# NVIDIA/DALI

Measured on NVIDIA B200. Metric: images/sec decode+resize+CMN (batch 256, 1080p JPEG), higher is better.
Workload: dtype u8

## Files before the change

dali_b200/csrc/common.cuh:

```cuda
#ifndef DALI_B200_CSRC_COMMON_CUH_
#define DALI_B200_CSRC_COMMON_CUH_

#include <cuda_runtime.h>
#include <cuda_fp16.h>
#include <stdint.h>
#include <atomic>
#include <cstdio>
#include <cstdarg>
#include <string>
#include <vector>
#include "../../include/dali_b200.h"

namespace dalib200 {

void SetLastError(const char *fmt, ...);
extern std::atomic<uint64_t> g_launch_count;
inline void CountLaunch(int n = 1) { g_launch_count.fetch_add(n, std::memory_order_relaxed); }

#define DB_CHECK_ARG(cond, ...)                                   \
  do { if (!(cond)) { ::dalib200::SetLastError(__VA_ARGS__); return DALIB200_ERROR_INVALID_ARGUMENT; } } while (0)

#define DB_CUDA(call)                                                                           \
  do { cudaError_t e__ = (call); if (e__ != cudaSuccess) {                                      \
    ::dalib200::SetLastError("CUDA error %s at %s:%d (%s)", cudaGetErrorName(e__), __FILE__, __LINE__, \
// ... 61 lines not shown

__device__ __forceinline__ float u8_to_float(uint32_t b) { return __uint_as_float(0x4B000000u | b) - 8388608.0f; }

template <typename T> struct OutConv;
template <> struct OutConv<float> {
  __device__ __forceinline__ static float cvt(float v) { return v; }
};
template <> struct OutConv<uint16_t> {
  __device__ __forceinline__ static uint16_t cvt(float v) { return float2half_ties_away(v); }
};

__device__ __forceinline__ float mul_rn(float a, float b) { return __fmul_rn(a, b); }
__device__ __forceinline__ float add_rn(float a, float b) { return __fadd_rn(a, b); }
__device__ __forceinline__ float sub_rn(float a, float b) { return __fsub_rn(a, b); }

__device__ __forceinline__ uint32_t ld_nc_u32(const uint32_t *p) {
  uint32_t v;
  asm volatile("ld.global.nc.u32 %0, [%1];" : "=r"(v) : "l"(p));
  return v;
}

__device__ __forceinline__ uint32_t smem_u32(const void *p) { return (uint32_t)__cvta_generic_to_shared(p); }
__device__ __forceinline__ uint32_t lds_u32(uint32_t a) { uint32_t v; asm volatile("ld.shared.u32 %0, [%1];" : "=r"(v) : "r"(a)); return v; }
__device__ __forceinline__ uint32_t lds_u16(uint32_t a) { unsigned short v; asm volatile("ld.shared.u16 %0, [%1];" : "=h"(v) : "r"(a)); return v; }
__device__ __forceinline__ uint32_t lds_u8(uint32_t a) { uint32_t v; asm volatile("ld.shared.u8 %0, [%1];" : "=r"(v) : "r"(a)); return v; }
__device__ __forceinline__ void sts_u32(uint32_t a, uint32_t v) { asm volatile("st.shared.u32 [%0], %1;" :: "r"(a), "r"(v) : "memory"); }
__device__ __forceinline__ void sts_u16(uint32_t a, uint32_t v) { asm volatile("st.shared.u16 [%0], %1;" :: "r"(a), "h"((unsigned short)v) : "memory"); }

__device__ __forceinline__ void mbar_init(uint64_t *bar, uint32_t count) {
  asm volatile("mbarrier.init.shared::cta.b64 [%0], %1;" :: "r"(smem_u32(bar)), "r"(count) : "memory");
}
__device__ __forceinline__ void mbar_expect_tx(uint64_t *bar, uint32_t bytes) {
  asm volatile("mbarrier.arrive.expect_tx.shared::cta.b64 _, [%0], %1;" :: "r"(smem_u32(bar)), "r"(bytes) : "memory");
}
__device__ __forceinline__ void mbar_arrive(uint64_t *bar) {
  asm volatile("mbarrier.arrive.shared::cta.b64 _, [%0];" :: "r"(smem_u32(bar)) : "memory");
}
__device__ __forceinline__ void mbar_wait(uint64_t *bar, uint32_t parity) {
  asm volatile("{\n\t.reg .pred p;\n\tWAIT_%=:\n\tmbarrier.try_wait.parity.shared::cta.b64 p, [%0], %1;\n\t@p bra DONE_%=;\n\tbra WAIT_%=;\n\tDONE_%=:\n\t}"
               :: "r"(smem_u32(bar)), "r"(parity) : "memory");
}
__device__ __forceinline__ void mbar_wait_backoff(uint64_t *bar, uint32_t parity) {
  uint32_t done = 0;
  for (;;) {
    asm volatile("{\n\t.reg .pred p;\n\tmbarrier.try_wait.parity.shared::cta.b64 p, [%1], %2;\n\tselp.u32 %0, 1, 0, p;\n\t}"
                 : "=r"(done) : "r"(smem_u32(bar)), "r"(parity) : "memory");
    if (done) break;
// ... 35 lines not shown
```

dali_b200/csrc/jpeg.cu:

```cuda
#include "common.cuh"
#include <algorithm>
#include <cstring>
#include <map>
#include <thread>

namespace dalib200 {

constexpr int kDcLutBits = 9, kAcLutBits = 11;
constexpr int kDcLutSize = 1 << kDcLutBits, kAcLutSize = 1 << kAcLutBits;
constexpr int kLutWords = 2 * kDcLutSize + 2 * kAcLutSize;
constexpr int kSyncThreads = 256;
constexpr int kChunkBytes = 4096;
constexpr int kMaxBlocksPerMcu = 10;
constexpr int kMaxLog2Sub = 10;

constexpr int kLongLut = 512;
struct HuffSlow {
  int32_t maxcode[18];
  int32_t valoff[18];
  uint8_t vals[256];
  int32_t long_base, long_n;
  uint16_t long_lut[kLongLut];
};

struct TableSet {
  uint32_t lut[kLutWords];
  uint16_t lut16[kLutWords];
  HuffSlow slow[4];
};
__host__ __device__ inline int LutOffset(int t) { return t < 2 ? t * kDcLutSize : 2 * kDcLutSize + (t - 2) * kAcLutSize; }

struct QuantSet { uint16_t q[4][64]; };

struct JpegImage {
  uint8_t *out;
  int32_t width, height, ncomp;
  int32_t hs[3], vs[3], hmax, vmax;
  int32_t mcux, mcuy, bpm;
  int32_t blk_comp[kMaxBlocksPerMcu];
  int32_t blk_dc[kMaxBlocksPerMcu], blk_ac[kMaxBlocksPerMcu];
  int32_t blk_x[kMaxBlocksPerMcu], blk_y[kMaxBlocksPerMcu];
  int32_t tq[3];
  int32_t restart_interval;
  int32_t table_set, quant_set;
  int32_t unit_begin, unit_end;
  int32_t subseq_begin;
  int32_t nsub;
  int32_t block_begin;
  int32_t wblock_begin;
// ... 182 lines not shown
    uint32_t *cw32 = reinterpret_cast<uint32_t *>(clean) + (out_base >> 2);
    for (uint32_t wd = threadIdx.x; wd < nwords; wd += blockDim.x) {
      const uint32_t v = obuf[wd];
      const bool full = (wd > 0 || head == 0) && (wd + 1 < nwords || tailb == 0);
      if (full) {
        cw32[wd] = __byte_perm(v, 0u, 0x0123);
      } else {
        const uint32_t lo = wd == 0 ? head : 0u, hi = (wd + 1 == nwords && tailb) ? tailb : 4u;
        for (uint32_t b = lo; b < hi; b++) reinterpret_cast<uint8_t *>(cw32 + wd)[3u - b] = (uint8_t)(v >> (8 * b));
      }
    }
    if (c0 + kChunkBytes >= u.raw_len) {
      const uint32_t e0 = out_base + total, e1 = u.clean_off + ((u.raw_len + 32u + 15u) & ~15u);
      for (uint32_t q = e0 + threadIdx.x; q < e1; q += blockDim.x) clean[(q & ~3u) | (3u - (q & 3u))] = 0;
    }
    __syncthreads();
  }
}

struct SmemSrc {
  uint32_t base; int lsw;
  __device__ __forceinline__ uint32_t load(uint32_t g) const { return lds_u32(base + ((g ^ ((g >> lsw) & 31u)) << 2)); }
};
struct SmemLut { uint32_t base; __device__ __forceinline__ uint32_t load(uint32_t i) const { return lds_u32(base + (i << 2)); } };
struct GlobalLut { const uint32_t *p; __device__ __forceinline__ uint32_t load(uint32_t i) const { return __ldg(p + i); } };
template <int STRIDE> struct SmemTbl { uint32_t base; __device__ __forceinline__ uint32_t load(int c) const { return lds_u32(base + (uint32_t)c * (STRIDE * 4u)); } };
struct GlobalSrc {
  const uint32_t *w;
  __device__ __forceinline__ uint32_t load(uint32_t g) const { return __ldg(w + g); }
};

template <class Src>
struct BitWindow {
  uint32_t hi, lo, g;
  int avail;
  __device__ __forceinline__ void init(const Src &s, uint32_t word, uint32_t sh) {
    const uint32_t w0 = s.load(word), w1 = s.load(word + 1);
    hi = __funnelshift_l(w1, w0, sh);
    lo = w1 << sh;
    avail = 64 - (int)sh;
    g = word + 2;
  }
  __device__ __forceinline__ void consume(const Src &s, uint32_t e) {
    hi = __funnelshift_l(lo, hi, e);
    lo = __funnelshift_l(0u, lo, e);
    avail -= (int)(e & 31u);
    const uint32_t w = s.load(g);
    const bool need = avail < 32;
    const uint32_t a = (uint32_t)avail & 31u;
    hi |= (need ? w : 0u) >> a;
    lo = need ? (w << ((32u - a) & 31u)) : lo;
    avail += need ? 32 : 0;
    g += need ? 1u : 0u;
  }
};

constexpr uint64_t kStateMask = (1ull << 42) - 1;
constexpr uint32_t kMaxChainLen = 4095;
__device__ __forceinline__ uint64_t pack_state(uint32_t p, int c, int z, uint32_t cnt = 0, uint32_t t = 0) {
  return (uint64_t)p | ((uint64_t)(uint32_t)c << 32) | ((uint64_t)(uint32_t)z << 36) | ((uint64_t)min(cnt, 1023u) << 42) | ((uint64_t)t << 52);
}
__device__ __forceinline__ uint32_t state_count(uint64_t s) { return (uint32_t)(s >> 42) & 1023u; }

__device__ __forceinline__ uint32_t make_entry(uint32_t len, uint32_t sym, bool is_dc) {
  const uint32_t s = sym & 15u, r = sym >> 4;
  const uint32_t adv = is_dc ? 1u : (s == 0 ? (r == 15u ? 16u : 64u) : r + 1u);
  return (len + s) | (s << 8) | (len << 12) | (adv << 20);
}

__device__ __forceinline__ uint32_t make_entry16(uint32_t len, uint32_t sym, bool is_dc) {
  const uint32_t s = sym & 15u, r = sym >> 4;
  const uint32_t adv = is_dc ? 1u : (s == 0 ? (r == 15u ? 16u : 64u) : r + 1u);
  return (len + s) | (s << 5) | (adv << 9);
}

__device__ __noinline__ uint32_t slow_lookup(const HuffSlow *__restrict__ slow, uint32_t toff, uint32_t hi, bool is_dc) {
  const int tbl = toff < 2u * kDcLutSize ? (int)(toff / kDcLutSize) : 2 + (int)((toff - 2u * kDcLutSize) / kAcLutSize);
  const HuffSlow *sl = slow + tbl;
  const int32_t code16 = (int32_t)(hi >> 16);
  if (sl->long_n > 0) {
    const int idx = min(max(code16 - sl->long_base, 0), sl->long_n - 1);
    const uint32_t e = sl->long_lut[idx];
    return e ? e : 16u;
  }
  uint32_t len = (is_dc ? kDcLutBits : kAcLutBits) + 1;
  while (len <= 16 && code16 >= sl->maxcode[len]) len++;
  uint32_t sym = 0;
  if (len > 16) len = 16;
  else sym = sl->vals[(sl->valoff[len] + (code16 >> (16 - len))) & 0xFF];
  return len | (sym << 8);
}
__device__ __forceinline__ uint32_t slow_symbol(const HuffSlow *__restrict__ slow, uint32_t toff, uint32_t hi, bool is_dc) {
  const uint32_t ls = slow_lookup(slow, toff, hi, is_dc);
  return make_entry(ls & 0xFFu, ls >> 8, is_dc);
}
__device__ __forceinline__ uint32_t slow_symbol16(const HuffSlow *__restrict__ slow, uint32_t toff, uint32_t hi, bool is_dc) {
  const uint32_t ls = slow_lookup(slow, toff, hi, is_dc);
  return make_entry16(ls & 0xFFu, ls >> 8, is_dc);
}

template <class Src, class Lut, class Tbl>
__device__ __forceinline__ void decode_span(const Src &src, BitWindow<Src> &win, const Lut &lut, const HuffSlow *__restrict__ slow,
                                            const Tbl &tbl, int bpm, uint32_t &pos, uint32_t end, int &c, int &z, uint32_t &nb) {
  uint32_t tb12 = tbl.load(c);
  while (pos < end) {
    const uint32_t e_ac = lut.load((tb12 >> 16) + (win.hi >> (32 - kAcLutBits)));
    const bool is_dc = z == 0;
    uint32_t e = e_ac;
    if (is_dc) e = lut.load((tb12 & 0xFFFFu) + (win.hi >> (32 - kDcLutBits)));
    if (__builtin_expect(e == 0, 0)) e = slow_symbol(slow, is_dc ? (tb12 & 0xFFFFu) : (tb12 >> 16), win.hi, is_dc);
    const uint32_t tb = e & 31u, adv = e >> 20;
    win.consume(src, e);
    pos += tb;
    z += (int)adv;
    const bool endb = z >= 64;
    const int c1 = c + 1 == bpm ? 0 : c + 1;
    nb += endb ? 1u : 0u;
    c = endb ? c1 : c;
    z = endb ? 0 : z;
    if (endb) tb12 = tbl.load(c);
  }
}

__device__ __forceinline__ int find_unit_by_subseq(const JpegUnit *u, int ub, int ue, int j) {
  int lo = ub, hi = ue - 1;
  while (lo < hi) {
    int mid = (lo + hi + 1) >> 1;
    if (u[mid].first_subseq <= j) lo = mid; else hi = mid - 1;
  }
  return lo;
}

struct HuffCtx {
  const JpegImage *images; int nimages;
  const int32_t *block_image;
  const int32_t *wblock_image;
  const JpegUnit *units;
  const uint32_t *unit_clean_len;
  const TableSet *tables;
  const uint8_t *clean;
  uint64_t *s_state;
  uint32_t *s_n;
  int16_t *coef;
  int16_t *dc;
  int log2_sub;
  int32_t *status;
  uint32_t *unit_nblk;
  uint4 *chains[3];
  uint32_t *chain_count;
};

__device__ __forceinline__ uint32_t tbl_word(const JpegImage &im, int b) {
  return (uint32_t)LutOffset(im.blk_dc[b]) | ((uint32_t)LutOffset(im.blk_ac[b]) << 16);
}

struct SyncSmem {
  uint32_t *lut, *sw, *cnt, *tbl, *col_end, *blkbuf;
  uint64_t *exitst;
  const uint8_t **colptr;
  uint8_t *zig, *col_cont;
  HuffSlow *slow;
};
constexpr int kMaxLookAheadCols = 8;
__host__ __device__ inline int look_ahead_cols(int log2_sub) { return 256 >> (log2_sub - 3); }
__host__ __device__ inline size_t sync_sw_words(int log2_sub) { return (size_t)(kSyncThreads + look_ahead_cols(log2_sub)) << (log2_sub - 5); }
__host__ __device__ inline size_t sync_smem_bytes(int log2_sub, bool with_block_buffers) {
  return kLutWords * 4 + sync_sw_words(log2_sub) * 4 + kSyncThreads * 8  + (kSyncThreads + kMaxLookAheadCols) * 8  +
         kSyncThreads * 4 * 2  + 16 * 4  + 64  + kSyncThreads  + 4 * sizeof(HuffSlow) +
         (with_block_buffers ? (size_t)kSyncThreads * 128 : 0) ;
}
__device__ __forceinline__ SyncSmem carve_sync_smem(uint32_t *base, int log2_sub) {
  SyncSmem s;
  s.lut = base;
  s.sw = s.lut + kLutWords;
  s.exitst = reinterpret_cast<uint64_t *>(s.sw + sync_sw_words(log2_sub));
  s.colptr = reinterpret_cast<const uint8_t **>(s.exitst + kSyncThreads);
  s.cnt = reinterpret_cast<uint32_t *>(s.colptr + kSyncThreads + kMaxLookAheadCols);
  s.col_end = s.cnt + kSyncThreads;
  s.tbl = s.col_end + kSyncThreads;
  s.zig = reinterpret_cast<uint8_t *>(s.tbl + 16);
  s.col_cont = s.zig + 64;
  s.slow = reinterpret_cast<HuffSlow *>(s.col_cont + kSyncThreads);
  s.blkbuf = reinterpret_cast<uint32_t *>(s.slow + 4);
  return s;
}

struct SubGeom { bool valid; int ui; uint32_t jl, nsub_eff, clean_bits; int64_t g; };

__device__ __forceinline__ SubGeom sync_block_prologue(const HuffCtx &cx, const JpegImage &im, const SyncSmem &sm) {
  const int lsw = cx.log2_sub - 5;
  {
    const uint4 *src = reinterpret_cast<const uint4 *>(cx.tables[im.table_set].lut);
    uint4 *dst = reinterpret_cast<uint4 *>(sm.lut);
    for (int i = threadIdx.x; i < kLutWords / 4; i += blockDim.x) dst[i] = __ldg(src + i);
    if (threadIdx.x < kMaxBlocksPerMcu) sm.tbl[threadIdx.x] = tbl_word(im, threadIdx.x);
    if (threadIdx.x < 64) sm.zig[threadIdx.x] = c_zigzag[threadIdx.x];
    const uint32_t *ssrc = reinterpret_cast<const uint32_t *>(cx.tables[im.table_set].slow);
    uint32_t *sdst = reinterpret_cast<uint32_t *>(sm.slow);
    for (int i = threadIdx.x; i < (int)(4 * sizeof(HuffSlow) / 4); i += blockDim.x) sdst[i] = __ldg(ssrc + i);
  }
  SubGeom sg;
  const int j = (blockIdx.x - im.block_begin) * kSyncThreads + threadIdx.x;
  sg.valid = j < im.nsub;
  sg.ui = 0; sg.jl = 0; sg.nsub_eff = 0; sg.clean_bits = 0;
  sg.g = (int64_t)im.subseq_begin + j;
  const uint8_t *ptr = nullptr;
  if (sg.valid) {
    sg.ui = im.unit_end - im.unit_begin == 1 ? im.unit_begin : find_unit_by_subseq(cx.units, im.unit_begin, im.unit_end, j);
    const JpegUnit &u = cx.units[sg.ui];
    sg.clean_bits = cx.unit_clean_len[sg.ui] * 8u;
    sg.nsub_eff = (sg.clean_bits + (1u << cx.log2_sub) - 1) >> cx.log2_sub;
    sg.jl = (uint32_t)(j - u.first_subseq);
    sg.valid = sg.jl < sg.nsub_eff;
    if (sg.valid) ptr = cx.clean + u.clean_off + ((size_t)sg.jl << (cx.log2_sub - 3));
  }
  sm.colptr[threadIdx.x] = ptr;
  sm.col_end[threadIdx.x] = min((sg.jl + 1) << cx.log2_sub, sg.clean_bits);
// ... 49 lines not shown
      const uint32_t x = threadIdx.x + 1;
      nb = 0;
      decode_span(src, win, lut, slow, tbl, im.bpm, pos, sm.col_end[x], c, z, nb);
      const uint64_t ns = pack_state(pos, c, z);
      const bool same = sm.exitst[x] == ns;
      sm.exitst[x] = ns; sm.cnt[x] = nb;
      if (!same && sm.col_cont[x]) push_chain(cx, 0, pos, c, z, 2u, sg.g + 2, img_i);
    }
  }
  __syncthreads();
  if (sg.valid) {
    const uint32_t t = threadIdx.x > 0 && sm.col_cont[threadIdx.x - 1] ? 1u : 0u;
    cx.s_state[sg.g] = sm.exitst[threadIdx.x] | ((uint64_t)min(sm.cnt[threadIdx.x], 1023u) << 42) | ((uint64_t)t << 52);
  }
}

constexpr int kTailThreads = 256;
constexpr int kTailColWords = 36;
struct ColSrc {
  uint32_t base;
  __device__ __forceinline__ uint32_t load(uint32_t g) const { return lds_u32(base + g * (kTailThreads * 4u)); }
};

__device__ __forceinline__ void walk_chain(const HuffCtx &cx, const uint4 rec, int out_list, int max_visits, const uint32_t *s_lut,
                                           const HuffSlow *s_slow, int s_table_set, uint32_t *col, uint32_t *tblcol) {
  const int img_i = (int)rec.w;
  const JpegImage &im = cx.images[img_i];
  int64_t g = rec.z;
  const int j = (int)(g - im.subseq_begin);
  const int ui = im.unit_end - im.unit_begin == 1 ? im.unit_begin : find_unit_by_subseq(cx.units, im.unit_begin, im.unit_end, j);
  const JpegUnit &u = cx.units[ui];
  const uint32_t clean_bits = cx.unit_clean_len[ui] * 8u;
  const uint32_t nsub_eff = (clean_bits + (1u << cx.log2_sub) - 1) >> cx.log2_sub;
  uint32_t jl = (uint32_t)(j - u.first_subseq);
#pragma unroll
  for (int b = 0; b < kMaxBlocksPerMcu; b++) tblcol[b * kTailThreads] = tbl_word(im, b);
  const bool shared_tables = im.table_set == s_table_set;
  uint32_t pos = rec.x, t = rec.y >> 16;
  int c = (int)(rec.y & 0xFF), z = (int)((rec.y >> 8) & 0xFF);
  const int sub_words = 1 << (cx.log2_sub - 5);
  for (int visit = 0;;) {
    uint32_t nb = 0;
    const uint32_t end = min((jl + 1) << cx.log2_sub, clean_bits);
    if (shared_tables && sub_words + 4 <= kTailColWords) {
      const uint4 *p4 = reinterpret_cast<const uint4 *>(cx.clean + u.clean_off + ((size_t)jl << (cx.log2_sub - 3)));
      for (int q = 0; q < sub_words / 4 + 1; q++) {
        const uint4 v = __ldg(p4 + q);
        col[(4 * q + 0) * kTailThreads] = v.x; col[(4 * q + 1) * kTailThreads] = v.y;
        col[(4 * q + 2) * kTailThreads] = v.z; col[(4 * q + 3) * kTailThreads] = v.w;
      }
      const ColSrc src{smem_u32(col)};
      const uint32_t rel = pos - (jl << cx.log2_sub);
      BitWindow<ColSrc> win;
      win.init(src, rel >> 5, rel & 31u);
      decode_span(src, win, SmemLut{smem_u32(s_lut)}, s_slow, SmemTbl<kTailThreads>{smem_u32(tblcol)}, im.bpm, pos, end, c, z, nb);
    } else {
      const GlobalSrc src{reinterpret_cast<const uint32_t *>(cx.clean + u.clean_off)};
      BitWindow<GlobalSrc> win;
      win.init(src, pos >> 5, pos & 31u);
      decode_span(src, win, GlobalLut{cx.tables[im.table_set].lut}, cx.tables[im.table_set].slow, SmemTbl<kTailThreads>{smem_u32(tblcol)},
                  im.bpm, pos, end, c, z, nb);
    }
    const uint64_t ns = pack_state(pos, c, z, nb, t);
    const uint64_t old = atomicMax(reinterpret_cast<unsigned long long *>(cx.s_state + g), (unsigned long long)ns);
    if ((uint32_t)(old >> 52) >= t) break;
    if (((old ^ ns) & kStateMask) == 0) break;
    if (jl + 1 >= nsub_eff || t >= kMaxChainLen) break;
    g++; jl++; t++;
    if (++visit >= max_visits) { push_chain(cx, out_list, pos, c, z, t, g, img_i); break; }
  }
}

__global__ void __launch_bounds__(kTailThreads) huff_sync_walk_kernel(HuffCtx cx, int in_list, int out_list, int max_visits) {
  extern __shared__ __align__(16) uint32_t tsm[];
  const uint32_t n = cx.chain_count[in_list];
  if (blockIdx.x * blockDim.x >= n) return;
  uint32_t *s_lut = tsm;
  HuffSlow *s_slow = reinterpret_cast<HuffSlow *>(s_lut + kLutWords);
  uint32_t *col = reinterpret_cast<uint32_t *>(s_slow + 4) + threadIdx.x;
  uint32_t *tblcol = reinterpret_cast<uint32_t *>(s_slow + 4) + kTailColWords * kTailThreads + threadIdx.x;
  const int s_table_set = cx.images[0].table_set;
  {
    const uint4 *src = reinterpret_cast<const uint4 *>(cx.tables[s_table_set].lut);
    uint4 *dst = reinterpret_cast<uint4 *>(s_lut);
    for (int i = threadIdx.x; i < kLutWords / 4; i += blockDim.x) dst[i] = __ldg(src + i);
    const uint32_t *ssrc = reinterpret_cast<const uint32_t *>(cx.tables[s_table_set].slow);
    uint32_t *sdst = reinterpret_cast<uint32_t *>(s_slow);
    for (int i = threadIdx.x; i < (int)(4 * sizeof(HuffSlow) / 4); i += blockDim.x) sdst[i] = __ldg(ssrc + i);
  }
  __syncthreads();
  const uint32_t gtid = blockIdx.x * blockDim.x + threadIdx.x, gsize = gridDim.x * blockDim.x;
  for (uint32_t i = gtid; i < n; i += gsize) walk_chain(cx, cx.chains[in_list][i], out_list, max_visits, s_lut, s_slow, s_table_set, col, tblcol);
}

__global__ void __launch_bounds__(1024) huff_scan_kernel(HuffCtx cx) {
  __shared__ uint32_t warp_tot[32];
  __shared__ uint32_t carry;
  const JpegImage &im = cx.images[blockIdx.x];
  const uint32_t sub_bits = 1u << cx.log2_sub;
  for (int ui = im.unit_begin; ui < im.unit_end; ui++) {
    const JpegUnit &u = cx.units[ui];
    const uint32_t clean_bits = cx.unit_clean_len[ui] * 8u;
    const uint32_t nsub_eff = (clean_bits + sub_bits - 1) >> cx.log2_sub;
    const int64_t g0 = (int64_t)im.subseq_begin + u.first_subseq;
    __syncthreads();
    if (threadIdx.x == 0) carry = 0;
    __syncthreads();
    for (uint32_t base = 0; base < nsub_eff; base += blockDim.x) {
// ... 3 lines not shown
      for (int o = 1; o < 32; o <<= 1) { uint32_t x = __shfl_up_sync(0xffffffffu, incl, o); if ((threadIdx.x & 31) >= o) incl += x; }
      if ((threadIdx.x & 31) == 31) warp_tot[threadIdx.x >> 5] = incl;
      __syncthreads();
      uint32_t woff = 0, tot = 0;
      for (int w = 0; w < (int)(blockDim.x >> 5); w++) { if (w < (int)(threadIdx.x >> 5)) woff += warp_tot[w]; tot += warp_tot[w]; }
      if (i < nsub_eff) cx.s_n[g0 + i] = carry + woff + incl - v;
      __syncthreads();
      if (threadIdx.x == 0) carry += tot;
      __syncthreads();
    }
    if (threadIdx.x == 0) {
      if ((int64_t)carry * 64 < u.nslots) cx.status[blockIdx.x] = 1;
      cx.unit_nblk[ui] = (uint32_t)min((int64_t)carry, u.nslots >> 6);
    }
  }
}

constexpr int kWriteThreads = 384;
struct WriteSmem {
  uint16_t *lut; uint32_t *sw, *tbl, *blkbuf; uint8_t *zig; HuffSlow *slow; const uint8_t **colptr;
};
__host__ __device__ inline size_t write_sw_words(int log2_sub) { return (size_t)(kWriteThreads + look_ahead_cols(log2_sub)) << (log2_sub - 5); }
__host__ __device__ inline size_t write_smem_bytes(int log2_sub) {
  return kLutWords * 2 + write_sw_words(log2_sub) * 4 + 16 * 4  + 64  + (size_t)kWriteThreads * 128;
}
__device__ __forceinline__ WriteSmem carve_write_smem(uint32_t *base, int log2_sub) {
  WriteSmem s;
  s.lut = reinterpret_cast<uint16_t *>(base);
  s.sw = base + kLutWords / 2;
  s.tbl = s.sw + write_sw_words(log2_sub);
  s.zig = reinterpret_cast<uint8_t *>(s.tbl + 16);
  s.slow = nullptr;
  s.blkbuf = reinterpret_cast<uint32_t *>(s.zig + 64);
  s.colptr = reinterpret_cast<const uint8_t **>(s.blkbuf);
  return s;
}

__global__ void __launch_bounds__(kWriteThreads) huff_write_kernel(HuffCtx cx) {
  extern __shared__ __align__(16) uint32_t hsm[];
  const WriteSmem sm = carve_write_smem(hsm, cx.log2_sub);
  const JpegImage &im = cx.images[cx.wblock_image[blockIdx.x]];
  const int lsw = cx.log2_sub - 5;
  {
    const uint4 *src = reinterpret_cast<const uint4 *>(cx.tables[im.table_set].lut16);
    uint4 *dst = reinterpret_cast<uint4 *>(sm.lut);
    for (int i = threadIdx.x; i < kLutWords * 2 / 16; i += blockDim.x) dst[i] = __ldg(src + i);
    if (threadIdx.x < kMaxBlocksPerMcu) sm.tbl[threadIdx.x] = tbl_word(im, threadIdx.x);
    if (threadIdx.x < 64) sm.zig[threadIdx.x] = c_zigzag[threadIdx.x];
  }
  SubGeom sg;
  {
    const int j = (blockIdx.x - im.wblock_begin) * kWriteThreads + threadIdx.x;
    sg.valid = j < im.nsub;
    sg.ui = 0; sg.jl = 0; sg.nsub_eff = 0; sg.clean_bits = 0;
    sg.g = (int64_t)im.subseq_begin + j;
    const uint8_t *ptr = nullptr;
    if (sg.valid) {
      sg.ui = im.unit_end - im.unit_begin == 1 ? im.unit_begin : find_unit_by_subseq(cx.units, im.unit_begin, im.unit_end, j);
      const JpegUnit &u = cx.units[sg.ui];
      sg.clean_bits = cx.unit_clean_len[sg.ui] * 8u;
      sg.nsub_eff = (sg.clean_bits + (1u << cx.log2_sub) - 1) >> cx.log2_sub;
      sg.jl = (uint32_t)(j - u.first_subseq);
      sg.valid = sg.jl < sg.nsub_eff;
      if (sg.valid) ptr = cx.clean + u.clean_off + ((size_t)sg.jl << (cx.log2_sub - 3));
    }
    sm.colptr[threadIdx.x] = ptr;
    const int la_cols = look_ahead_cols(cx.log2_sub);
    if (threadIdx.x == kWriteThreads - 1)
      for (int q = 1; q <= la_cols; q++) sm.colptr[kWriteThreads - 1 + q] = ptr ? ptr + ((size_t)q << (cx.log2_sub - 3)) : nullptr;
    __syncthreads();
    const int cpc = 1 << (cx.log2_sub - 7);
    for (int ch = threadIdx.x; ch < (kWriteThreads + la_cols) * cpc; ch += blockDim.x) {
      const int col = ch / cpc, o = ch - col * cpc;
      const uint8_t *p = sm.colptr[col];
      if (p) {
        const uint4 v = __ldg(reinterpret_cast<const uint4 *>(p) + o);
        const uint32_t g = ((uint32_t)col << lsw) + 4u * o, x = (uint32_t)col & 31u;
        sm.sw[(g + 0) ^ x] = v.x; sm.sw[(g + 1) ^ x] = v.y; sm.sw[(g + 2) ^ x] = v.z; sm.sw[(g + 3) ^ x] = v.w;
      }
    }
    __syncthreads();
  }
  const HuffSlow *slow = cx.tables[im.table_set].slow;
  const SmemSrc src{smem_u32(sm.sw), lsw};
  const uint32_t lane = threadIdx.x & 31u;
  const uint32_t a_lut = smem_u32(sm.lut), a_tbl = smem_u32(sm.tbl), a_zig = smem_u32(sm.zig);
  const uint32_t a_wbuf = smem_u32(sm.blkbuf) + (threadIdx.x & ~31u) * 128u;
  const uint32_t a_mybuf = a_wbuf + lane * 128u;
#pragma unroll
  for (int j = 0; j < 32; j++) sts_u32(a_mybuf + 4u * j, 0u);
  __syncwarp();
  uint32_t pos = 0, nb = 0, end = 0, hard_end = 0, blk0 = 0, blk_limit = 0;
  int c = 0, z = 0;
  bool active = sg.valid;
  if (active) {
    const JpegUnit &u = cx.units[sg.ui];
    if (sg.jl > 0) {
      const uint64_t prev = cx.s_state[sg.g - 1];
      pos = (uint32_t)prev; c = (int)((prev >> 32) & 15u); z = (int)((prev >> 36) & 63u);
    }
    end = min((sg.jl + 1) << cx.log2_sub, sg.clean_bits);
    hard_end = sg.clean_bits;
    const uint32_t ublk = (uint32_t)(u.slot_base >> 6);
    blk0 = ublk + cx.s_n[sg.g];
    blk_limit = ublk + (uint32_t)(u.nslots >> 6);
    active = pos < end && blk0 < blk_limit;
  }
  bool own = z == 0;
  BitWindow<SmemSrc> win;
  {
    const uint32_t rel = active ? pos - (sg.jl << cx.log2_sub) : 0u;
    win.init(src, ((uint32_t)threadIdx.x << lsw) + (rel >> 5), rel & 31u);
  }
  int16_t *coef = cx.coef + im.coef_off;
  int16_t *dcv = cx.dc + im.coef_off / 64;
  const int bpm = im.bpm;
  uint32_t tb12 = lds_u32(a_tbl + 4u * c);
  while (__any_sync(0xffffffffu, active)) {
    bool flush = false;
    const uint32_t blk = blk0 + nb;
    if (active) {
      const uint32_t e_ac = lds_u16(a_lut + 2u * ((tb12 >> 16) + (win.hi >> (32 - kAcLutBits))));
      const bool is_dc = z == 0;
      uint32_t e = e_ac;
      if (is_dc) e = lds_u16(a_lut + 2u * ((tb12 & 0xFFFFu) + (win.hi >> (32 - kDcLutBits))));
      if (__builtin_expect(e == 0, 0)) e = slow_symbol16(slow, is_dc ? (tb12 & 0xFFFFu) : (tb12 >> 16), win.hi, is_dc);
      const uint32_t tb = e & 31u, adv = e >> 9, s = (e >> 5) & 15u;
      {
        const uint32_t len = tb - s;
        const uint32_t bits = (uint32_t)(((uint64_t)(win.hi << len)) >> (32u - s));
        const int v = (int)bits - ((s == 0 || ((bits >> (s - 1u)) & 1u)) ? 0 : (int)((1u << s) - 1u));
        if (own) {
          if (is_dc) {
            dcv[blk] = (int16_t)v;
          } else if (s) {
            const uint32_t nat = lds_u8(a_zig + min((uint32_t)z + adv - 1u, 63u));
            sts_u16(a_mybuf + 4u * ((nat >> 1) ^ lane) + 2u * (nat & 1u), (uint32_t)v);
          }
        }
      }
      win.consume(src, e);
      pos += tb;
      z += (int)adv;
      const bool endb = z >= 64;
      const int c1 = c + 1 == bpm ? 0 : c + 1;
      flush = endb && own;
      nb += endb ? 1u : 0u;
      own = own || endb;
      c = endb ? c1 : c;
      z = endb ? 0 : z;
      if (endb) tb12 = lds_u32(a_tbl + 4u * c);
      active = blk0 + nb < blk_limit && (pos < end || (z != 0 && pos < hard_end));
    }
    uint32_t m = __ballot_sync(0xffffffffu, flush);
    while (m) {
      const uint32_t L = __ffs(m) - 1u;
      m &= m - 1u;
      const uint32_t fb = __shfl_sync(0xffffffffu, blk, L);
      const uint32_t a_src = a_wbuf + L * 128u + 4u * (lane ^ L);
      const uint32_t w = lds_u32(a_src);
      sts_u32(a_src, 0u);
      reinterpret_cast<uint32_t *>(coef + (size_t)fb * 64)[lane] = w;
    }
    __syncwarp();
  }
}

__global__ void __launch_bounds__(1024) dc_scan_kernel(const JpegImage *__restrict__ images, int16_t *__restrict__ dc_arena) {
  __shared__ int warp_tot[32];
  const JpegImage &im = images[blockIdx.x];
  int16_t *dc = dc_arena + im.coef_off / 64;
  const int nmcu = im.mcux * im.mcuy;
  const int ri = im.restart_interval > 0 ? im.restart_interval : nmcu;
  const int lane = threadIdx.x & 31, wid = threadIdx.x >> 5;
  for (int comp = 0; comp < im.ncomp; comp++) {
    int nb = 0, bidx[kMaxBlocksPerMcu];
    for (int b = 0; b < im.bpm; b++) if (im.blk_comp[b] == comp) bidx[nb++] = b;
    const int total = nmcu * nb;
    if (ri >= nmcu) {
      const int per = ((total + 31) / 32 + 31) / 32 * 32;
      const int i0 = wid * per, i1 = min(total, i0 + per);
      int sum = 0;
      for (int i = i0 + lane; i < i1; i += 32) sum += dc[(i / nb) * im.bpm + bidx[i % nb]];
      for (int o = 16; o; o >>= 1) sum += __shfl_xor_sync(0xffffffffu, sum, o);
      __syncthreads();
// ... 631 lines not shown
        j.scan_comp[i] = ci; j.td[i] = s[2 + 2 * i] >> 4; j.ta[i] = s[2 + 2 * i] & 15;
      }
      j.scan_begin = pos + L;
      break;
    }
    pos += L;
    if (!need_scan && got_sof && m == 0xC0 + (j.progressive ? 2 : 0)) {
    }
  }
  if (!got_sof) { SetLastError("JPEG: no frame header found"); return DALIB200_ERROR_BAD_DATA; }
  if (j.width == 0 || j.height == 0) { SetLastError("JPEG: zero image size"); return DALIB200_ERROR_BAD_DATA; }
  if (need_scan && !j.scan_begin) { SetLastError("JPEG: no scan found"); return DALIB200_ERROR_BAD_DATA; }
  return DALIB200_SUCCESS;
}

void FillInfo(const ParsedJpeg &j, dalib200JpegInfo *info) {
  info->width = j.width; info->height = j.height;
  info->components = j.ncomp;
  info->subsampling = (j.hs[0] << 4) | j.vs[0];
  info->restart_interval = j.restart_interval;
  info->orientation = j.orientation;
}

uint32_t MakeLutEntry(int len, int sym, bool is_dc) {
  const uint32_t s = sym & 15, r = (uint32_t)sym >> 4;
  const uint32_t adv = is_dc ? 1u : (s == 0 ? (r == 15u ? 16u : 64u) : r + 1u);
  return ((uint32_t)len + s) | (s << 8) | ((uint32_t)len << 12) | (adv << 20);
}

uint16_t MakeLutEntry16(int len, int sym, bool is_dc) {
  const uint32_t s = sym & 15, r = (uint32_t)sym >> 4;
  const uint32_t adv = is_dc ? 1u : (s == 0 ? (r == 15u ? 16u : 64u) : r + 1u);
  return (uint16_t)(((uint32_t)len + s) | (s << 5) | (adv << 9));
}

void BuildDeviceTable(const HostHuff &h, uint32_t *lut, uint16_t *lut16, HuffSlow &t, bool is_dc) {
  const int kLutBits = is_dc ? kDcLutBits : kAcLutBits, kLutSize = 1 << kLutBits;
  memset(&t, 0, sizeof(t));
  memset(lut, 0, sizeof(uint32_t) * kLutSize);
  memset(lut16, 0, sizeof(uint16_t) * kLutSize);
  int code = 0, k = 0;
  for (int l = 1; l <= 16; l++) {
    const int mincode = code;
    t.valoff[l] = k - mincode;
    for (int i = 0; i < h.bits[l]; i++, k++, code++) {
      if (l <= kLutBits) {
        const int lo = code << (kLutBits - l), cnt = 1 << (kLutBits - l);
        for (int e = 0; e < cnt && lo + e < kLutSize; e++) {
          lut[lo + e] = MakeLutEntry(l, h.vals[k & 255], is_dc);
          lut16[lo + e] = MakeLutEntry16(l, h.vals[k & 255], is_dc);
        }
      }
    }
    t.maxcode[l] = code << (16 - l);
    code <<= 1;
  }
  t.maxcode[17] = 0x7fffffff;
  memcpy(t.vals, h.vals, 256);
  t.long_base = t.maxcode[kLutBits];
  const int range = 65536 - t.long_base;
  t.long_n = 0;
  if (range > 0 && range <= kLongLut) {
    t.long_n = range;
    int c2 = 0, k2 = 0;
    for (int l = 1; l <= 16; l++) {
      for (int i = 0; i < h.bits[l]; i++, k2++, c2++) {
        if (l > kLutBits) {
          const int lo = (c2 << (16 - l)) - t.long_base, cnt = 1 << (16 - l);
          for (int e = 0; e < cnt; e++)
            if (lo + e >= 0 && lo + e < range) t.long_lut[lo + e] = (uint16_t)(l | (h.vals[k2 & 255] << 8));
        }
      }
      c2 <<= 1;
    }
// ... 286 lines not shown
      if (j.td[si] > 1 || j.ta[si] > 1) return unsupported("Huffman table ids above 1 are not supported (baseline allows 0..1)");
      if (!prog && (!j.dc[j.td[si]].present || !j.ac[j.ta[si]].present)) { SetLastError("decoders.image: sample %d: missing Huffman table", i); return DALIB200_ERROR_BAD_DATA; }
      for (int v = 0; v < j.vs[c]; v++)
        for (int h = 0; h < j.hs[c]; h++) {
          if (bpm >= kMaxBlocksPerMcu) return unsupported("too many blocks per MCU");
          im.blk_comp[bpm] = c; im.blk_dc[bpm] = j.td[si]; im.blk_ac[bpm] = 2 + j.ta[si]; im.blk_x[bpm] = h; im.blk_y[bpm] = v;
          bpm++;
        }
    }
    im.bpm = bpm;
    {
      std::string key;
      if (prog) key = "progressive";
      else
      for (int t = 0; t < 2; t++) { key.append(reinterpret_cast<const char *>(j.dc[t].bits), 17); key.append(reinterpret_cast<const char *>(j.dc[t].vals), 256); key.push_back(j.dc[t].present); }
      if (!prog)
      for (int t = 0; t < 2; t++) { key.append(reinterpret_cast<const char *>(j.ac[t].bits), 17); key.append(reinterpret_cast<const char *>(j.ac[t].vals), 256); key.push_back(j.ac[t].present); }
      auto it = table_cache.find(key);
      if (it == table_cache.end()) {
        TableSet ts;
        if (prog) memset(&ts, 0, sizeof(ts));
        else
        for (int t = 0; t < 2; t++) {
          BuildDeviceTable(j.dc[t], ts.lut + LutOffset(t), ts.lut16 + LutOffset(t), ts.slow[t], true);
          BuildDeviceTable(j.ac[t], ts.lut + LutOffset(2 + t), ts.lut16 + LutOffset(2 + t), ts.slow[2 + t], false);
        }
        p->tables.push_back(ts);
        it = table_cache.emplace(key, (int)p->tables.size() - 1).first;
      }
      im.table_set = it->second;
      std::string qk(reinterpret_cast<const char *>(j.qt), sizeof(j.qt));
      auto qi = quant_cache.find(qk);
      if (qi == quant_cache.end()) {
        QuantSet qs; memcpy(qs.q, j.qt, sizeof(j.qt));
        p->quants.push_back(qs);
        qi = quant_cache.emplace(qk, (int)p->quants.size() - 1).first;
      }
      im.quant_set = qi->second;
    }
    const uint8_t *d = streams[i];
    size_t sb = j.scan_begin, se = lengths[i];
    if (se >= sb + 2 && d[se - 2] == 0xFF && d[se - 1] == 0xD9) se -= 2;
    j.scan_end = se;
    const int64_t nmcu = (int64_t)im.mcux * im.mcuy;
    im.unit_begin = (int)p->units.size();
    im.subseq_begin = (int)subseq;
    im.block_begin = sync_blocks;
    im.wblock_begin = write_blocks;
// ... 408 lines not shown
    a.d_first_blk = reinterpret_cast<const int64_t *>(p->prog_arena.dev + o_blk);
    a.total_blocks = p->prog_total_blocks;
    a.wave_begin = &p->prog_wave_begin; a.h_images = &p->prog_images;
    a.d_raw = d_raw; a.d_coef = p->d_coef; a.d_dc = p->d_dc; a.d_status = p->d_status;
    if ((rc = LaunchProgressive(a, ps))) return rc;
    DB_CUDA(cudaEventRecord(p->prog_join, ps));
  }
  const bool any_units = nunits > 0 && p->nchunks > 0 && p->total_blocks_sync > 0;
  if (any_units) {
    const int grid = (int)std::min<uint32_t>(p->nchunks, (uint32_t)sms * 16);
    { ProfScope ps_("jpeg_unstuff_count", s); unstuff_count_kernel<<<grid, 256, 0, s>>>(d_raw, d_units, nunits, p->nchunks, p->d_chunk); }
    { ProfScope ps_("jpeg_unstuff_scan", s); unstuff_scan_kernel<<<(nunits + 7) / 8, 256, 0, s>>>(d_units, nunits, p->d_chunk, p->d_unit_len); }
    { ProfScope ps_("jpeg_unstuff_scatter", s); unstuff_scatter_kernel<<<grid, 256, 0, s>>>(d_raw, d_units, nunits, p->nchunks, p->d_chunk, p->d_clean); }
    CountLaunch(3);
  }
  HuffCtx cx;
  cx.images = d_images; cx.nimages = p->n; cx.block_image = reinterpret_cast<const int32_t *>(p->d_stage + p->off_blkimg);
  cx.wblock_image = reinterpret_cast<const int32_t *>(p->d_stage + p->off_wblkimg);
  cx.units = d_units; cx.unit_clean_len = p->d_unit_len; cx.tables = d_tables;
  cx.clean = p->d_clean; cx.s_state = p->d_state; cx.s_n = p->d_n; cx.coef = p->d_coef; cx.dc = p->d_dc; cx.log2_sub = p->log2_sub;
  cx.status = p->d_status; cx.unit_nblk = p->d_unit_nblk;
  cx.chains[0] = p->d_chain1; cx.chains[1] = p->d_chain2; cx.chains[2] = p->d_chain3; cx.chain_count = p->d_chain_count;
  const size_t hsmem = sync_smem_bytes(p->log2_sub, false), wsmem = write_smem_bytes(p->log2_sub);
  const size_t walk_smem = kLutWords * 4 + 4 * sizeof(HuffSlow) + (size_t)(kTailColWords + kMaxBlocksPerMcu) * kTailThreads * 4;
  if (!p->smem_opted) {
    DB_CUDA(cudaFuncSetAttribute(huff_sync_intra_kernel, cudaFuncAttributeMaxDynamicSharedMemorySize, (int)sync_smem_bytes(kMaxLog2Sub, false)));
    DB_CUDA(cudaFuncSetAttribute(huff_write_kernel, cudaFuncAttributeMaxDynamicSharedMemorySize, (int)write_smem_bytes(kMaxLog2Sub)));
    DB_CUDA(cudaFuncSetAttribute(huff_sync_walk_kernel, cudaFuncAttributeMaxDynamicSharedMemorySize, (int)walk_smem));
    int per_sm = 0;
    DB_CUDA(cudaOccupancyMaxActiveBlocksPerMultiprocessor(&per_sm, huff_sync_walk_kernel, kTailThreads, walk_smem));
    p->walk_max_grid = std::max(1, per_sm) * sms * 4;
    p->smem_opted = true;
  }
  if (any_units) { ProfScope ps_("jpeg_huff_sync_intra", s); huff_sync_intra_kernel<<<p->total_blocks_sync, kSyncThreads, hsmem, s>>>(cx); }
  if (any_units) {
    auto walk_grid = [&](double frac) {
      const int64_t want = (int64_t)(p->total_subseq * frac) / kTailThreads + p->total_blocks_sync / kTailThreads + 1;
      return (int)std::max<int64_t>(1, std::min<int64_t>(p->walk_max_grid, want));
    };
    { ProfScope ps_("jpeg_huff_sync_walk1", s); huff_sync_walk_kernel<<<walk_grid(0.40), kTailThreads, walk_smem, s>>>(cx, 0, 1, 1); }
    { ProfScope ps_("jpeg_huff_sync_walk2", s); huff_sync_walk_kernel<<<walk_grid(0.14), kTailThreads, walk_smem, s>>>(cx, 1, 2, 1); }
    { ProfScope ps_("jpeg_huff_sync_walk3", s); huff_sync_walk_kernel<<<walk_grid(0.06), kTailThreads, walk_smem, s>>>(cx, 2, 0, 1 << 30); }
    CountLaunch(2);
  }
  { ProfScope ps_("jpeg_huff_scan", s); huff_scan_kernel<<<p->n, 1024, 0, s>>>(cx); }
  CountLaunch();
  if (any_units && p->total_blocks_write > 0) { ProfScope ps_("jpeg_huff_write", s); huff_write_kernel<<<p->total_blocks_write, kWriteThreads, wsmem, s>>>(cx); }
// ... 34 lines not shown
```

Before: 45030.

## Switch Huffman sync/walk LUTs to 16-bit entries and streamline write-kernel coefficient store

Drops the 32-bit Huffman lookup table and makes the sync and walk kernels use the existing 16-bit packed entries. This halves LUT shared memory and the per-block copy cost, which may allow higher occupancy. The write kernel now uses a precomputed zigzag table holding doubled byte offsets with a one-slot shift, and a simpler branch-light sign extension. DC values are recovered from the flushed coefficient word instead of a separate store. It also reads the smem base from a stored word so address arithmetic stays in shared space. The risk is correctness coupling between the new zigzag indexing and the DC handling.

```diff
diff --git a/dali_b200/csrc/common.cuh b/dali_b200/csrc/common.cuh
--- a/dali_b200/csrc/common.cuh
+++ b/dali_b200/csrc/common.cuh
@@ -107,7 +107,7 @@
 
 __device__ __forceinline__ uint32_t smem_u32(const void *p) { return (uint32_t)__cvta_generic_to_shared(p); }
 __device__ __forceinline__ uint32_t lds_u32(uint32_t a) { uint32_t v; asm volatile("ld.shared.u32 %0, [%1];" : "=r"(v) : "r"(a)); return v; }
-__device__ __forceinline__ uint32_t lds_u16(uint32_t a) { unsigned short v; asm volatile("ld.shared.u16 %0, [%1];" : "=h"(v) : "r"(a)); return v; }
+__device__ __forceinline__ uint32_t lds_u16(uint32_t a) { uint32_t v; asm volatile("ld.shared.u16 %0, [%1];" : "=r"(v) : "r"(a)); return v; }
 __device__ __forceinline__ uint32_t lds_u8(uint32_t a) { uint32_t v; asm volatile("ld.shared.u8 %0, [%1];" : "=r"(v) : "r"(a)); return v; }
 __device__ __forceinline__ void sts_u32(uint32_t a, uint32_t v) { asm volatile("st.shared.u32 [%0], %1;" :: "r"(a), "r"(v) : "memory"); }
 __device__ __forceinline__ void sts_u16(uint32_t a, uint32_t v) { asm volatile("st.shared.u16 [%0], %1;" :: "r"(a), "h"((unsigned short)v) : "memory"); }
diff --git a/dali_b200/csrc/jpeg.cu b/dali_b200/csrc/jpeg.cu
--- a/dali_b200/csrc/jpeg.cu
+++ b/dali_b200/csrc/jpeg.cu
@@ -24,7 +24,6 @@
 };
 
 struct TableSet {
-  uint32_t lut[kLutWords];
   uint16_t lut16[kLutWords];
   HuffSlow slow[4];
 };
@@ -253,8 +252,8 @@
   uint32_t base; int lsw;
   __device__ __forceinline__ uint32_t load(uint32_t g) const { return lds_u32(base + ((g ^ ((g >> lsw) & 31u)) << 2)); }
 };
-struct SmemLut { uint32_t base; __device__ __forceinline__ uint32_t load(uint32_t i) const { return lds_u32(base + (i << 2)); } };
-struct GlobalLut { const uint32_t *p; __device__ __forceinline__ uint32_t load(uint32_t i) const { return __ldg(p + i); } };
+struct SmemLut { uint32_t base; __device__ __forceinline__ uint32_t load(uint32_t i) const { return lds_u16(base + (i << 1)); } };
+struct GlobalLut { const uint16_t *p; __device__ __forceinline__ uint32_t load(uint32_t i) const { return __ldg(p + i); } };
 template <int STRIDE> struct SmemTbl { uint32_t base; __device__ __forceinline__ uint32_t load(int c) const { return lds_u32(base + (uint32_t)c * (STRIDE * 4u)); } };
 struct GlobalSrc {
   const uint32_t *w;
@@ -293,12 +292,6 @@
 }
 __device__ __forceinline__ uint32_t state_count(uint64_t s) { return (uint32_t)(s >> 42) & 1023u; }
 
-__device__ __forceinline__ uint32_t make_entry(uint32_t len, uint32_t sym, bool is_dc) {
-  const uint32_t s = sym & 15u, r = sym >> 4;
-  const uint32_t adv = is_dc ? 1u : (s == 0 ? (r == 15u ? 16u : 64u) : r + 1u);
-  return (len + s) | (s << 8) | (len << 12) | (adv << 20);
-}
-
 __device__ __forceinline__ uint32_t make_entry16(uint32_t len, uint32_t sym, bool is_dc) {
   const uint32_t s = sym & 15u, r = sym >> 4;
   const uint32_t adv = is_dc ? 1u : (s == 0 ? (r == 15u ? 16u : 64u) : r + 1u);
@@ -320,10 +313,6 @@
   if (len > 16) len = 16;
   else sym = sl->vals[(sl->valoff[len] + (code16 >> (16 - len))) & 0xFF];
   return len | (sym << 8);
-}
-__device__ __forceinline__ uint32_t slow_symbol(const HuffSlow *__restrict__ slow, uint32_t toff, uint32_t hi, bool is_dc) {
-  const uint32_t ls = slow_lookup(slow, toff, hi, is_dc);
-  return make_entry(ls & 0xFFu, ls >> 8, is_dc);
 }
 __device__ __forceinline__ uint32_t slow_symbol16(const HuffSlow *__restrict__ slow, uint32_t toff, uint32_t hi, bool is_dc) {
   const uint32_t ls = slow_lookup(slow, toff, hi, is_dc);
@@ -339,8 +328,8 @@
     const bool is_dc = z == 0;
     uint32_t e = e_ac;
     if (is_dc) e = lut.load((tb12 & 0xFFFFu) + (win.hi >> (32 - kDcLutBits)));
-    if (__builtin_expect(e == 0, 0)) e = slow_symbol(slow, is_dc ? (tb12 & 0xFFFFu) : (tb12 >> 16), win.hi, is_dc);
-    const uint32_t tb = e & 31u, adv = e >> 20;
+    if (__builtin_expect(e == 0, 0)) e = slow_symbol16(slow, is_dc ? (tb12 & 0xFFFFu) : (tb12 >> 16), win.hi, is_dc);
+    const uint32_t tb = e & 31u, adv = e >> 9;
     win.consume(src, e);
     pos += tb;
     z += (int)adv;
@@ -386,7 +375,8 @@
 }
 
 struct SyncSmem {
-  uint32_t *lut, *sw, *cnt, *tbl, *col_end, *blkbuf;
+  uint16_t *lut;
+  uint32_t *sw, *cnt, *tbl, *col_end, *blkbuf;
   uint64_t *exitst;
   const uint8_t **colptr;
   uint8_t *zig, *col_cont;
@@ -396,14 +386,14 @@
 __host__ __device__ inline int look_ahead_cols(int log2_sub) { return 256 >> (log2_sub - 3); }
 __host__ __device__ inline size_t sync_sw_words(int log2_sub) { return (size_t)(kSyncThreads + look_ahead_cols(log2_sub)) << (log2_sub - 5); }
 __host__ __device__ inline size_t sync_smem_bytes(int log2_sub, bool with_block_buffers) {
-  return kLutWords * 4 + sync_sw_words(log2_sub) * 4 + kSyncThreads * 8  + (kSyncThreads + kMaxLookAheadCols) * 8  +
+  return kLutWords * 2 + sync_sw_words(log2_sub) * 4 + kSyncThreads * 8  + (kSyncThreads + kMaxLookAheadCols) * 8  +
          kSyncThreads * 4 * 2  + 16 * 4  + 64  + kSyncThreads  + 4 * sizeof(HuffSlow) +
          (with_block_buffers ? (size_t)kSyncThreads * 128 : 0) ;
 }
 __device__ __forceinline__ SyncSmem carve_sync_smem(uint32_t *base, int log2_sub) {
   SyncSmem s;
-  s.lut = base;
-  s.sw = s.lut + kLutWords;
+  s.lut = reinterpret_cast<uint16_t *>(base);
+  s.sw = base + kLutWords / 2;
   s.exitst = reinterpret_cast<uint64_t *>(s.sw + sync_sw_words(log2_sub));
   s.colptr = reinterpret_cast<const uint8_t **>(s.exitst + kSyncThreads);
   s.cnt = reinterpret_cast<uint32_t *>(s.colptr + kSyncThreads + kMaxLookAheadCols);
@@ -421,9 +411,9 @@
 __device__ __forceinline__ SubGeom sync_block_prologue(const HuffCtx &cx, const JpegImage &im, const SyncSmem &sm) {
   const int lsw = cx.log2_sub - 5;
   {
-    const uint4 *src = reinterpret_cast<const uint4 *>(cx.tables[im.table_set].lut);
+    const uint4 *src = reinterpret_cast<const uint4 *>(cx.tables[im.table_set].lut16);
     uint4 *dst = reinterpret_cast<uint4 *>(sm.lut);
-    for (int i = threadIdx.x; i < kLutWords / 4; i += blockDim.x) dst[i] = __ldg(src + i);
+    for (int i = threadIdx.x; i < kLutWords * 2 / 16; i += blockDim.x) dst[i] = __ldg(src + i);
     if (threadIdx.x < kMaxBlocksPerMcu) sm.tbl[threadIdx.x] = tbl_word(im, threadIdx.x);
     if (threadIdx.x < 64) sm.zig[threadIdx.x] = c_zigzag[threadIdx.x];
     const uint32_t *ssrc = reinterpret_cast<const uint32_t *>(cx.tables[im.table_set].slow);
@@ -519,7 +509,7 @@
   __device__ __forceinline__ uint32_t load(uint32_t g) const { return lds_u32(base + g * (kTailThreads * 4u)); }
 };
 
-__device__ __forceinline__ void walk_chain(const HuffCtx &cx, const uint4 rec, int out_list, int max_visits, const uint32_t *s_lut,
+__device__ __forceinline__ void walk_chain(const HuffCtx &cx, const uint4 rec, int out_list, int max_visits, const uint16_t *s_lut,
                                            const HuffSlow *s_slow, int s_table_set, uint32_t *col, uint32_t *tblcol) {
   const int img_i = (int)rec.w;
   const JpegImage &im = cx.images[img_i];
@@ -555,7 +545,7 @@
       const GlobalSrc src{reinterpret_cast<const uint32_t *>(cx.clean + u.clean_off)};
       BitWindow<GlobalSrc> win;
       win.init(src, pos >> 5, pos & 31u);
-      decode_span(src, win, GlobalLut{cx.tables[im.table_set].lut}, cx.tables[im.table_set].slow, SmemTbl<kTailThreads>{smem_u32(tblcol)},
+      decode_span(src, win, GlobalLut{cx.tables[im.table_set].lut16}, cx.tables[im.table_set].slow, SmemTbl<kTailThreads>{smem_u32(tblcol)},
                   im.bpm, pos, end, c, z, nb);
     }
     const uint64_t ns = pack_state(pos, c, z, nb, t);
@@ -572,15 +562,15 @@
   extern __shared__ __align__(16) uint32_t tsm[];
   const uint32_t n = cx.chain_count[in_list];
   if (blockIdx.x * blockDim.x >= n) return;
-  uint32_t *s_lut = tsm;
+  uint16_t *s_lut = reinterpret_cast<uint16_t *>(tsm);
   HuffSlow *s_slow = reinterpret_cast<HuffSlow *>(s_lut + kLutWords);
   uint32_t *col = reinterpret_cast<uint32_t *>(s_slow + 4) + threadIdx.x;
   uint32_t *tblcol = reinterpret_cast<uint32_t *>(s_slow + 4) + kTailColWords * kTailThreads + threadIdx.x;
   const int s_table_set = cx.images[0].table_set;
   {
-    const uint4 *src = reinterpret_cast<const uint4 *>(cx.tables[s_table_set].lut);
+    const uint4 *src = reinterpret_cast<const uint4 *>(cx.tables[s_table_set].lut16);
     uint4 *dst = reinterpret_cast<uint4 *>(s_lut);
-    for (int i = threadIdx.x; i < kLutWords / 4; i += blockDim.x) dst[i] = __ldg(src + i);
+    for (int i = threadIdx.x; i < kLutWords * 2 / 16; i += blockDim.x) dst[i] = __ldg(src + i);
     const uint32_t *ssrc = reinterpret_cast<const uint32_t *>(cx.tables[s_table_set].slow);
     uint32_t *sdst = reinterpret_cast<uint32_t *>(s_slow);
     for (int i = threadIdx.x; i < (int)(4 * sizeof(HuffSlow) / 4); i += blockDim.x) sdst[i] = __ldg(ssrc + i);
@@ -630,7 +620,7 @@
 };
 __host__ __device__ inline size_t write_sw_words(int log2_sub) { return (size_t)(kWriteThreads + look_ahead_cols(log2_sub)) << (log2_sub - 5); }
 __host__ __device__ inline size_t write_smem_bytes(int log2_sub) {
-  return kLutWords * 2 + write_sw_words(log2_sub) * 4 + 16 * 4  + 64  + (size_t)kWriteThreads * 128;
+  return kLutWords * 2 + write_sw_words(log2_sub) * 4 + 16 * 4  + 128  + (size_t)kWriteThreads * 128;
 }
 __device__ __forceinline__ WriteSmem carve_write_smem(uint32_t *base, int log2_sub) {
   WriteSmem s;
@@ -639,7 +629,7 @@
   s.tbl = s.sw + write_sw_words(log2_sub);
   s.zig = reinterpret_cast<uint8_t *>(s.tbl + 16);
   s.slow = nullptr;
-  s.blkbuf = reinterpret_cast<uint32_t *>(s.zig + 64);
+  s.blkbuf = reinterpret_cast<uint32_t *>(s.zig + 128);
   s.colptr = reinterpret_cast<const uint8_t **>(s.blkbuf);
   return s;
 }
@@ -654,7 +644,8 @@
     uint4 *dst = reinterpret_cast<uint4 *>(sm.lut);
     for (int i = threadIdx.x; i < kLutWords * 2 / 16; i += blockDim.x) dst[i] = __ldg(src + i);
     if (threadIdx.x < kMaxBlocksPerMcu) sm.tbl[threadIdx.x] = tbl_word(im, threadIdx.x);
-    if (threadIdx.x < 64) sm.zig[threadIdx.x] = c_zigzag[threadIdx.x];
+    if (threadIdx.x == 15) sm.tbl[15] = smem_u32(hsm);
+    if (threadIdx.x < 128) sm.zig[threadIdx.x] = (uint8_t)(2u * c_zigzag[min(max((int)threadIdx.x - 1, 0), 63)]);
   }
   SubGeom sg;
   {
@@ -690,11 +681,13 @@
     __syncthreads();
   }
   const HuffSlow *slow = cx.tables[im.table_set].slow;
-  const SmemSrc src{smem_u32(sm.sw), lsw};
   const uint32_t lane = threadIdx.x & 31u;
-  const uint32_t a_lut = smem_u32(sm.lut), a_tbl = smem_u32(sm.tbl), a_zig = smem_u32(sm.zig);
-  const uint32_t a_wbuf = smem_u32(sm.blkbuf) + (threadIdx.x & ~31u) * 128u;
-  const uint32_t a_mybuf = a_wbuf + lane * 128u;
+  const uint32_t a_base = lds_u32(smem_u32(sm.tbl + 15));
+  const auto at = [&](const void *p) { return a_base + (smem_u32(p) - smem_u32(hsm)); };
+  const uint32_t a_lut = at(sm.lut), a_tbl = at(sm.tbl), a_zig = at(sm.zig);
+  const uint32_t a_wbuf = at(sm.blkbuf) + (threadIdx.x & ~31u) * 128u;
+  const uint32_t a_mybuf = a_wbuf + lane * 128u, lane4 = lane << 2;
+  const SmemSrc src{at(sm.sw), lsw};
 #pragma unroll
   for (int j = 0; j < 32; j++) sts_u32(a_mybuf + 4u * j, 0u);
   __syncwarp();
@@ -734,18 +727,11 @@
       if (is_dc) e = lds_u16(a_lut + 2u * ((tb12 & 0xFFFFu) + (win.hi >> (32 - kDcLutBits))));
       if (__builtin_expect(e == 0, 0)) e = slow_symbol16(slow, is_dc ? (tb12 & 0xFFFFu) : (tb12 >> 16), win.hi, is_dc);
       const uint32_t tb = e & 31u, adv = e >> 9, s = (e >> 5) & 15u;
-      {
-        const uint32_t len = tb - s;
-        const uint32_t bits = (uint32_t)(((uint64_t)(win.hi << len)) >> (32u - s));
-        const int v = (int)bits - ((s == 0 || ((bits >> (s - 1u)) & 1u)) ? 0 : (int)((1u << s) - 1u));
-        if (own) {
-          if (is_dc) {
-            dcv[blk] = (int16_t)v;
-          } else if (s) {
-            const uint32_t nat = lds_u8(a_zig + min((uint32_t)z + adv - 1u, 63u));
-            sts_u16(a_mybuf + 4u * ((nat >> 1) ^ lane) + 2u * (nat & 1u), (uint32_t)v);
-          }
-        }
+      if (own && s) {
+        const uint32_t t = win.hi << (tb - s);
+        const uint32_t bits = __funnelshift_l(t, 0u, s);
+        const uint32_t v = bits + ((int)t < 0 ? 0u : 1u - (1u << s));
+        sts_u16(a_mybuf + (lds_u8(a_zig + (uint32_t)z + adv) ^ lane4), v);
       }
       win.consume(src, e);
       pos += tb;
@@ -765,10 +751,11 @@
       const uint32_t L = __ffs(m) - 1u;
       m &= m - 1u;
       const uint32_t fb = __shfl_sync(0xffffffffu, blk, L);
-      const uint32_t a_src = a_wbuf + L * 128u + 4u * (lane ^ L);
-      const uint32_t w = lds_u32(a_src);
-      sts_u32(a_src, 0u);
+      const uint32_t a_w = a_wbuf + L * 128u + 4u * (lane ^ L);
+      const uint32_t w = lds_u32(a_w);
+      sts_u32(a_w, 0u);
       reinterpret_cast<uint32_t *>(coef + (size_t)fb * 64)[lane] = w;
+      if (lane == 0) dcv[fb] = (int16_t)w;
     }
     __syncwarp();
   }
@@ -1446,22 +1433,15 @@
   info->orientation = j.orientation;
 }
 
-uint32_t MakeLutEntry(int len, int sym, bool is_dc) {
-  const uint32_t s = sym & 15, r = (uint32_t)sym >> 4;
-  const uint32_t adv = is_dc ? 1u : (s == 0 ? (r == 15u ? 16u : 64u) : r + 1u);
-  return ((uint32_t)len + s) | (s << 8) | ((uint32_t)len << 12) | (adv << 20);
-}
-
 uint16_t MakeLutEntry16(int len, int sym, bool is_dc) {
   const uint32_t s = sym & 15, r = (uint32_t)sym >> 4;
   const uint32_t adv = is_dc ? 1u : (s == 0 ? (r == 15u ? 16u : 64u) : r + 1u);
   return (uint16_t)(((uint32_t)len + s) | (s << 5) | (adv << 9));
 }
 
-void BuildDeviceTable(const HostHuff &h, uint32_t *lut, uint16_t *lut16, HuffSlow &t, bool is_dc) {
+void BuildDeviceTable(const HostHuff &h, uint16_t *lut16, HuffSlow &t, bool is_dc) {
   const int kLutBits = is_dc ? kDcLutBits : kAcLutBits, kLutSize = 1 << kLutBits;
   memset(&t, 0, sizeof(t));
-  memset(lut, 0, sizeof(uint32_t) * kLutSize);
   memset(lut16, 0, sizeof(uint16_t) * kLutSize);
   int code = 0, k = 0;
   for (int l = 1; l <= 16; l++) {
@@ -1470,10 +1450,7 @@
     for (int i = 0; i < h.bits[l]; i++, k++, code++) {
       if (l <= kLutBits) {
         const int lo = code << (kLutBits - l), cnt = 1 << (kLutBits - l);
-        for (int e = 0; e < cnt && lo + e < kLutSize; e++) {
-          lut[lo + e] = MakeLutEntry(l, h.vals[k & 255], is_dc);
-          lut16[lo + e] = MakeLutEntry16(l, h.vals[k & 255], is_dc);
-        }
+        for (int e = 0; e < cnt && lo + e < kLutSize; e++) lut16[lo + e] = MakeLutEntry16(l, h.vals[k & 255], is_dc);
       }
     }
     t.maxcode[l] = code << (16 - l);
@@ -1806,8 +1783,8 @@
         if (prog) memset(&ts, 0, sizeof(ts));
         else
         for (int t = 0; t < 2; t++) {
-          BuildDeviceTable(j.dc[t], ts.lut + LutOffset(t), ts.lut16 + LutOffset(t), ts.slow[t], true);
-          BuildDeviceTable(j.ac[t], ts.lut + LutOffset(2 + t), ts.lut16 + LutOffset(2 + t), ts.slow[2 + t], false);
+          BuildDeviceTable(j.dc[t], ts.lut16 + LutOffset(t), ts.slow[t], true);
+          BuildDeviceTable(j.ac[t], ts.lut16 + LutOffset(2 + t), ts.slow[2 + t], false);
         }
         p->tables.push_back(ts);
         it = table_cache.emplace(key, (int)p->tables.size() - 1).first;
@@ -2262,7 +2239,7 @@
   cx.status = p->d_status; cx.unit_nblk = p->d_unit_nblk;
   cx.chains[0] = p->d_chain1; cx.chains[1] = p->d_chain2; cx.chains[2] = p->d_chain3; cx.chain_count = p->d_chain_count;
   const size_t hsmem = sync_smem_bytes(p->log2_sub, false), wsmem = write_smem_bytes(p->log2_sub);
-  const size_t walk_smem = kLutWords * 4 + 4 * sizeof(HuffSlow) + (size_t)(kTailColWords + kMaxBlocksPerMcu) * kTailThreads * 4;
+  const size_t walk_smem = kLutWords * 2 + 4 * sizeof(HuffSlow) + (size_t)(kTailColWords + kMaxBlocksPerMcu) * kTailThreads * 4;
   if (!p->smem_opted) {
     DB_CUDA(cudaFuncSetAttribute(huff_sync_intra_kernel, cudaFuncAttributeMaxDynamicSharedMemorySize, (int)sync_smem_bytes(kMaxLog2Sub, false)));
     DB_CUDA(cudaFuncSetAttribute(huff_write_kernel, cudaFuncAttributeMaxDynamicSharedMemorySize, (int)write_smem_bytes(kMaxLog2Sub)));
```

Result: faster. 45540 (median of 6 runs) (+1.1%).
